# kawshik8/GAN-Image-Captioning

Measured on AMD Instinct MI355X. Metric: captions/sec (G+D train step), higher is better.
Workload: dtype bf16

## Files before the change

### gan-image-captioning_amd/csrc/gemm.hip

```cpp
#include "gemm.h"
#include "conv3x3.h"
#include "conv1x1_stream.h"
#include "conv1x1_panel.h"
#include "conv1x1_pix.h"
#include "conv_stem.h"
#include "bn_fold.h"
#include "kernels.h"

#include <stdlib.h>

namespace gic {

namespace {

typedef __attribute__((address_space(3))) bf16x4 lds_bf16x4;
typedef unsigned int u32x4 __attribute__((ext_vector_type(4)));
typedef const __attribute__((address_space(1))) u32x4* gptr_u4;

__device__ __attribute__((aligned(16))) unsigned int g_zero16[4] = {0u, 0u, 0u, 0u};
typedef __attribute__((address_space(3))) void* lds_void_ptr;
typedef const __attribute__((address_space(1))) void* gbl_void_ptr;

#ifdef GIC_STAMPS
}
__device__ unsigned long long g_stamp[32];
namespace {
#define STAMP(i) do { if (tid == 0 && blockIdx.y == 0 && (blockIdx.x == 0 || blockIdx.x == gridDim.x - 1)) { \
  const int o_ = blockIdx.x == 0 ? 0 : 16; g_stamp[o_ + 2 * (i)] = __builtin_amdgcn_s_memtime(); g_stamp[o_ + 2 * (i) + 1] = __builtin_amdgcn_s_memrealtime(); } } while (0)
#define DBG d.dbg
#else
#define STAMP(i) do {} while (0)
#define DBG 0
#endif

template <typename T> struct GlobalPtr { typedef const __attribute__((address_space(1))) T* type; };

template <typename TI, typename TO, bool AKC, bool BKC, int BM, int BN, bool VEC, int EPI, bool CONV, bool PIPE>
__global__ __launch_bounds__(256) void gemm_kernel(const GemmDesc d, const int k_tiles_per_split) {
  static_assert(!CONV || (AKC && BKC && VEC), "the implicit-GEMM convolution loader is k-contiguous and vectorised");
  static_assert(!PIPE || (AKC && BKC && VEC), "the LDS-DMA pipeline needs k-contiguous 16-byte chunks");
  constexpr int SZ = sizeof(TI);
  constexpr int BK = 128 / SZ;
  constexpr int VE = 16 / SZ;
  constexpr int SA = PIPE ? 128 : (AKC ? 144 : BM * SZ + 16);
  constexpr int SB = PIPE ? 128 : (BKC ? 144 : BN * SZ + 16);
  constexpr int NSTAGE = PIPE ? 3 : 2;
  constexpr int A_BYTES = AKC ? BM * SA : BK * SA;
  constexpr int B_BYTES = BKC ? BN * SB : BK * SB;
  constexpr int BUF_BYTES = A_BYTES + B_BYTES;
  constexpr int TM = BM / 32, TN = BN / 32;
  constexpr int CA = BM / 32, CB = BN / 32;
  constexpr bool IS_BF16 = (SZ == 2);
  typedef typename GlobalPtr<TI>::type gptr_t;

  constexpr int EPI_BYTES = BM * (BN * (int)sizeof(TO) + 16) + 4 * (BN / 2) * 2 * 4;
  constexpr int SMEM_BYTES = NSTAGE * BUF_BYTES > EPI_BYTES ? NSTAGE * BUF_BYTES : EPI_BYTES;
  __shared__ __attribute__((aligned(16))) unsigned char smem[SMEM_BYTES];

  const int tid = threadIdx.x, lane = tid & 63, w = tid >> 6;
  STAMP(0);
  const int wr = w >> 1, wc = w & 1;
  const int lr = lane & 15, lg = lane >> 4;

  const int tiles_m = (d.M + BM - 1) / BM;
  const int nwg = gridDim.x;
  int bid = blockIdx.x;
// ... 382 lines not shown
        if (m >= M) continue;
        float v = d.alpha * acc[i][j][r] + bias;
        if constexpr (EPI == EPI_BNSTATS) {
          C[(long)m * d.ldc + n] = from_f32<TO>(v);
          st_s += v; st_q += v * v;
        } else if constexpr (EPI == EPI_PLAIN) {
          const long o = (long)m * d.ldc + n;
          if constexpr (sizeof(TO) == 4) {
            if (split) { atomicAdd((float*)&C[o], v); continue; }
          }
          if (d.accumulate) v += to_f32<TO>(C[o]);
          C[o] = from_f32<TO>(v);
        } else {
          const float x = to_f32<TI>(((const TI*)d.X)[(long)m * d.ldx + n]);
          const float sg = 1.f / (1.f + expf(-v));
          const float y = sg * fmaxf(v, 0.f) + (1.f - sg) * x;
          if (d.Hpre) d.Hpre[(long)m * d.ldh + n] = v;
          float keep = keep4[r];
          if (d.mask) keep = (float)d.mask[(long)m * d.ldmask + n];
          if (d.mask_out) d.mask_out[(long)m * d.ldmask_out + n] = (uint8_t)keep;
          C[(long)m * d.ldc + n] = from_f32<TO>(y * keep * d.keep_scale);
        }
      }
      if constexpr (EPI == EPI_BNSTATS) {
        st_s += __shfl_xor(st_s, 16, 64); st_q += __shfl_xor(st_q, 16, 64);
        st_s += __shfl_xor(st_s, 32, 64); st_q += __shfl_xor(st_q, 32, 64);
        float* st = d.stats + (long)(blockIdx.x % d.stats_nrep) * 2 * N;
        if (lg == 0) { atomicAdd(&st[n], st_s); atomicAdd(&st[N + n], st_q); }
      }
    }
  }
}

template <typename TO, int BN, int EPI, bool CONV, int NS, bool ABN = false, bool ARES = false, int AMAXK = (ARES ? 2048 : 1024)>
__global__ __launch_bounds__(512) void tile8_kernel(const GemmDesc d, const unsigned a_bytes, const unsigned b_bytes) {
  static_assert(!ARES || ABN, "the residual-on-load form extends the A-side BatchNorm");
  constexpr int BM = 128, BK = 64, NT = 512;
  constexpr int TM = 2, TN = BN / 32;
  constexpr int CA = BM * 8 / NT, CB = BN * 8 / NT;
  constexpr int NL = CA + CB + (ARES ? CA : 0);
  constexpr int A_BYTES = BM * 128, B_BYTES = BN * 128, R_BYTES = ARES ? A_BYTES : 0, STAGE = A_BYTES + B_BYTES + R_BYTES;
  constexpr int OSZ = sizeof(TO), OVE = 16 / OSZ, SC = BN * OSZ + 16;
  constexpr int EPI_BYTES = EPI == EPI_HIGHWAY ? BM * (BN + 4) * 4 : (EPI == EPI_GUMBELMAX ? 8 * BN * 4 : BM * SC + 8 * (BN / 2) * 2 * 4);
  constexpr int RING_BYTES = NS * STAGE > EPI_BYTES ? NS * STAGE : EPI_BYTES;
  constexpr int ABN_MAXK = AMAXK;
  constexpr int SMEM_BYTES = RING_BYTES + (ABN ? ABN_MAXK * 8 : 0) + (ARES ? ABN_MAXK * 8 : 0);
  constexpr unsigned OOB = 0x80000000u;
  static_assert(CB >= 1 && SMEM_BYTES <= 160 * 1024, "tile8 LDS budget");
  __shared__ __attribute__((aligned(16))) unsigned char smem[SMEM_BYTES];

  const int tid = threadIdx.x, lane = tid & 63, w = tid >> 6;
  STAMP(0);
  const int wr = w >> 1, wc = w & 1;
  const int lr = lane & 15, lg = lane >> 4;

  const int tiles_m = (d.M + BM - 1) / BM, tiles_n = (d.N + BN - 1) / BN;
  const int bid = xcd_run(blockIdx.x, gridDim.x);
  const int bm0 = (d.n_fast ? bid / tiles_n : bid % tiles_m) * BM;
  const int bn0 = (d.n_fast ? bid % tiles_n : bid / tiles_m) * BN;
  const int M = d.M, N = d.N, K = d.K;

  const __amdgpu_buffer_rsrc_t rsA = __builtin_amdgcn_make_buffer_rsrc((void*)d.A, 0, (int)a_bytes, 0x00020000);
  const __amdgpu_buffer_rsrc_t rsB = __builtin_amdgcn_make_buffer_rsrc((void*)d.B, 0, (int)b_bytes, 0x00020000);
  const __amdgpu_buffer_rsrc_t rsR = __builtin_amdgcn_make_buffer_rsrc((void*)(ARES ? d.res : d.A), 0, (int)a_bytes, 0x00020000);

  const int kc = ((tid & 7) ^ ((tid >> 4) & 7)) * 8;
  int a_off[CA], a_hi0[CA], a_wi0[CA];
  bool a_ok[CA];
  int cv_r = 0, cv_s = 0, cv_c = 0;
#pragma unroll
  for (int i = 0; i < CA; ++i) {
    const int m = bm0 + (tid >> 3) + i * 64;
    a_ok[i] = m < M;
    if constexpr (CONV) {
      const int mm = a_ok[i] ? m : 0;
      const int wo = mm % d.cWo, t = mm / d.cWo;
      const int ho = t % d.cHo, n = t / d.cHo;
      a_hi0[i] = a_ok[i] ? ho * d.cStride - d.cPad : -(1 << 28);
      a_wi0[i] = wo * d.cStride - d.cPad;
      a_off[i] = ((n * d.cH + a_hi0[i]) * d.cW + a_wi0[i]) * d.cCin;
    } else {
      a_hi0[i] = a_wi0[i] = 0;
      a_off[i] = m * (int)d.lda;
    }
  }
  if constexpr (CONV) {
    cv_c = kc % d.cCin;
    const int t = kc / d.cCin;
    cv_s = t % d.cKW;
    cv_r = t / d.cKW;
  }
  int b_off[CB];
  bool b_ok[CB];
#pragma unroll
  for (int i = 0; i < CB; ++i) {
    const int n = bn0 + (tid >> 3) + i * 64;
    b_ok[i] = n < N;
    b_off[i] = n * (int)d.ldb;
  }
  const int wbase = (tid & ~63) * 16;

  auto issue = [&](int kt, int st) {
    unsigned char* sA = smem + st * STAGE;
    unsigned char* sB = sA + A_BYTES;
    const int k = kt * BK + kc;
    const bool kok = k < K;
#pragma unroll
    for (int i = 0; i < CA; ++i) {
      unsigned voff;
      if constexpr (CONV) {
        const bool ok = (unsigned)(a_hi0[i] + cv_r) < (unsigned)d.cH & (unsigned)(a_wi0[i] + cv_s) < (unsigned)d.cW & kok;
        voff = ok ? (unsigned)(a_off[i] + (cv_r * d.cW + cv_s) * d.cCin + cv_c) * 2u : OOB;
      } else {
        voff = (a_ok[i] & kok) ? (unsigned)(a_off[i] + k) * 2u : OOB;
      }
      __builtin_amdgcn_raw_ptr_buffer_load_lds(rsA, (lds_void_ptr)(sA + i * (NT * 16) + wbase), 16, (int)voff, 0, 0, CONV ? GIC_TRUNK_NT : 0);
      if constexpr (ARES)
        __builtin_amdgcn_raw_ptr_buffer_load_lds(rsR, (lds_void_ptr)(sB + B_BYTES + i * (NT * 16) + wbase), 16, (int)voff, 0, 0, CONV ? GIC_TRUNK_NT : 0);
    }
#pragma unroll
    for (int i = 0; i < CB; ++i) {
      const unsigned voff = (b_ok[i] & kok) ? (unsigned)(b_off[i] + k) * 2u : OOB;
      __builtin_amdgcn_raw_ptr_buffer_load_lds(rsB, (lds_void_ptr)(sB + i * (NT * 16) + wbase), 16, (int)voff, 0, 0, 0);
    }
    if constexpr (CONV) {
      cv_c += BK;
      while (cv_c >= d.cCin) {
        cv_c -= d.cCin;
        if (++cv_s == d.cKW) { cv_s = 0; ++cv_r; }
      }
    }
  };

  float* coef = (float*)(smem + RING_BYTES);
  if constexpr (ABN) {
    const int Cn = CONV ? d.cCin : K;
    for (int c = tid; c < ABN_MAXK; c += NT) {
      float sc = 0.f, sh = 0.f;
      if (c < Cn) {
        float s1, s2;
        fold_replicas(d.in_stats, d.in_nrep, Cn, c, s1, s2);
        const float mean = s1 * d.in_inv_count;
        const float var = fmaxf(s2 * d.in_inv_count - mean * mean, 0.f);
        sc = d.in_gamma[c] * rsqrtf(var + 1e-5f);
        sh = d.in_beta[c] - mean * sc;
      }
      coef[2 * c] = sc; coef[2 * c + 1] = sh;
      if constexpr (ARES) {
        float rs = 1.f, rt = 0.f;
        if (d.res_stats && c < Cn) {
          float s1, s2;
          fold_replicas(d.res_stats, d.res_nrep, Cn, c, s1, s2);
          const float mean = s1 * d.res_inv_count;
          const float var = fmaxf(s2 * d.res_inv_count - mean * mean, 0.f);
          rs = d.res_gamma[c] * rsqrtf(var + 1e-5f);
// ... 27 lines not shown
        for (int i = 0; i < CA; ++i) {
          const bool ok = CONV ? ((unsigned)(a_hi0[i] + tr) < (unsigned)d.cH & (unsigned)(a_wi0[i] + ts) < (unsigned)d.cW) : a_ok[i];
          if (!ok) continue;
          bf16x8* p = (bf16x8*)(smem + st * STAGE + i * (NT * 16) + tid * 16);
          bf16x8 v = *p;
          if constexpr (ARES) {
            const bf16x8 r = *(const bf16x8*)(smem + st * STAGE + A_BYTES + B_BYTES + i * (NT * 16) + tid * 16);
#pragma unroll
            for (int e = 0; e < 8; ++e) v[e] = (bf16_t)fmaxf((float)v[e] * scl[e] + sft[e] + ((float)r[e] * rsc[e] + rsf[e]), 0.f);
            if (wb) *(bf16x8*)((bf16_t*)d.out_wb + (long)a_off[i] + k) = v;
          } else {
#pragma unroll
            for (int e = 0; e < 8; ++e) v[e] = (bf16_t)fmaxf((float)v[e] * scl[e] + sft[e], 0.f);
          }
          *p = v;
        }
      }
    }
  };

  f32x4 acc[TM][TN];
#pragma unroll
  for (int i = 0; i < TM; ++i)
#pragma unroll
    for (int j = 0; j < TN; ++j) acc[i][j] = (f32x4){0.f, 0.f, 0.f, 0.f};

  auto compute = [&](int st) {
    const unsigned char* sA = smem + st * STAGE;
    const unsigned char* sB = sA + A_BYTES;
    bf16x8 fa[2][TM], fb[2][TN];
#pragma unroll
    for (int ks = 0; ks < 2; ++ks) {
#pragma unroll
      for (int t = 0; t < TM; ++t) {
        const int row = wr * 32 + t * 16 + lr;
        fa[ks][t] = *(const bf16x8*)(sA + row * 128 + (((ks * 4 + lg) ^ ((row >> 1) & 7)) << 4));
      }
#pragma unroll
      for (int t = 0; t < TN; ++t) {
        const int row = wc * (BN / 2) + t * 16 + lr;
        fb[ks][t] = *(const bf16x8*)(sB + row * 128 + (((ks * 4 + lg) ^ ((row >> 1) & 7)) << 4));
      }
    }
#pragma unroll
    for (int ks = 0; ks < 2; ++ks)
#pragma unroll
      for (int i = 0; i < TM; ++i)
#pragma unroll
        for (int j = 0; j < TN; ++j)
          acc[i][j] = __builtin_amdgcn_mfma_f32_16x16x32_bf16(fa[ks][i], fb[ks][j], acc[i][j], 0, 0, 0);
  };

  auto read_half = [&](int st, int ks, bf16x8 (&fa)[TM], bf16x8 (&fb)[TN]) {
    const unsigned char* sA = smem + st * STAGE;
    const unsigned char* sB = sA + A_BYTES;
#pragma unroll
    for (int t = 0; t < TM; ++t) {
      const int row = wr * 32 + t * 16 + lr;
      fa[t] = *(const bf16x8*)(sA + row * 128 + (((ks * 4 + lg) ^ ((row >> 1) & 7)) << 4));
    }
#pragma unroll
    for (int t = 0; t < TN; ++t) {
      const int row = wc * (BN / 2) + t * 16 + lr;
      fb[t] = *(const bf16x8*)(sB + row * 128 + (((ks * 4 + lg) ^ ((row >> 1) & 7)) << 4));
    }
  };
  auto mfma_half = [&](const bf16x8 (&fa)[TM], const bf16x8 (&fb)[TN]) {
#pragma unroll
    for (int i = 0; i < TM; ++i)
#pragma unroll
      for (int j = 0; j < TN; ++j)
        acc[i][j] = __builtin_amdgcn_mfma_f32_16x16x32_bf16(fa[i], fb[j], acc[i][j], 0, 0, 0);
  };

  const int nk = (K + BK - 1) / BK;
  STAMP(1);
  if constexpr (NS == 1) {
    for (int kt = 0; kt < nk; ++kt) {
      if (kt) __builtin_amdgcn_s_barrier();
      issue(kt, 0);
      asm volatile("s_waitcnt vmcnt(0)" ::: "memory");
      abn(kt, 0);
      __builtin_amdgcn_s_barrier();
      compute(0);
    }
  } else if constexpr (NS < 4) {
    issue(0, 0);
    int st = 0;
    for (int kt = 0; kt < nk; ++kt) {
      asm volatile("s_waitcnt vmcnt(0)" ::: "memory");
      abn(kt, st);
      __builtin_amdgcn_s_barrier();
      if (kt == 0) STAMP(2);
      if (!(DBG & 1)) issue(kt + 1, st ^ 1);
      if (!(DBG & 2)) compute(st);
      st ^= 1;
    }
  } else {
#pragma unroll
    for (int s = 0; s < NS - 1; ++s) issue(s, s);
    bf16x8 fa0[TM], fb0[TN], fa1[TM], fb1[TN];
    int st = 0, st_fill = NS - 1;
    for (int kt = 0; kt < nk; ++kt) {
      asm volatile("s_waitcnt vmcnt(%0) lgkmcnt(0)" ::"n"(NS >= 2 ? (NS - 2) * NL : 0) : "memory");
      abn(kt, st);
      __builtin_amdgcn_s_barrier();
      if (kt == 0) STAMP(2);
      if (!(DBG & 2)) {
        read_half(st, 0, fa0, fb0);
        __builtin_amdgcn_sched_barrier(0);
        if (kt > 0) mfma_half(fa1, fb1);
        __builtin_amdgcn_sched_barrier(0);
      }
      if (!(DBG & 1)) issue(kt + NS - 1, st_fill);
      if (!(DBG & 2)) {
        __builtin_amdgcn_sched_barrier(0);
        read_half(st, 1, fa1, fb1);
        __builtin_amdgcn_sched_barrier(0);
        mfma_half(fa0, fb0);
      }
      st = st == NS - 1 ? 0 : st + 1;
      st_fill = st_fill == NS - 1 ? 0 : st_fill + 1;
    }
    if (!(DBG & 2) && nk > 0) mfma_half(fa1, fb1);
  }
  asm volatile("s_waitcnt vmcnt(0)" ::: "memory");
  __syncthreads();
  STAMP(3);

  if constexpr (EPI == EPI_GUMBELMAX) {
    float* sV = (float*)smem;
    int* sI = (int*)(smem + 4 * BN * 4);
    const float eps = 1e-10f;
    const uint64_t seed = d.seed_dev ? *d.seed_dev : d.seed;
    const float T = d.gm_temperature;
#pragma unroll
    for (int j = 0; j < TN; ++j) {
      const int nl = wc * (BN / 2) + j * 16 + lr;
      const int n = bn0 + nl;
      float best = -INFINITY;
      int best_i = 0x7fffffff;
#pragma unroll
      for (int i = 0; i < TM; ++i) {
        const int m0 = bm0 + wr * 32 + i * 16 + lg * 4;
        if (m0 < M && n < N) {
          const float4 bv = *(const float4*)(d.gm_bias + m0);
          const float bia[4] = {bv.x, bv.y, bv.z, bv.w};
// ... 115 lines not shown
        if (!d.mask && d.use_philox) {
          uint32_t r0, r1, r2, r3;
          Philox::gen4(d.seed_dev ? *d.seed_dev : d.seed, d.stream, (uint64_t)(mb >> 2) * (uint64_t)N + (uint64_t)n, r0, r1, r2, r3);
          keep4[0] = Philox::u01(r0) >= d.drop_p ? 1.f : 0.f;
          keep4[1] = Philox::u01(r1) >= d.drop_p ? 1.f : 0.f;
          keep4[2] = Philox::u01(r2) >= d.drop_p ? 1.f : 0.f;
          keep4[3] = Philox::u01(r3) >= d.drop_p ? 1.f : 0.f;
        }
#pragma unroll
        for (int r = 0; r < 4; ++r) {
          const int m = mb + r;
          if (m >= M) continue;
          const float v = d.alpha * acc[i][j][r] + bias;
          const float x = to_f32<bf16_t>(((const bf16_t*)d.X)[(long)m * d.ldx + n]);
          const float sg = 1.f / (1.f + expf(-v));
          const float y = sg * fmaxf(v, 0.f) + (1.f - sg) * x;
          if (d.Hpre) d.Hpre[(long)m * d.ldh + n] = v;
          float keep = keep4[r];
          if (d.mask) keep = (float)d.mask[(long)m * d.ldmask + n];
          if (d.mask_out) d.mask_out[(long)m * d.ldmask_out + n] = (uint8_t)keep;
          C[(long)m * d.ldc + n] = from_f32<TO>(y * keep * d.keep_scale);
        }
      }
    }
    STAMP(5);
    return;
  }
  unsigned char* sC = smem;
  float* sStat = (float*)(smem + BM * SC);
#pragma unroll
  for (int j = 0; j < TN; ++j) {
    const int nl = wc * (BN / 2) + j * 16 + lr;
    const int n = bn0 + nl;
    const float bias = (d.bias && n < N) ? d.bias[n] : 0.f;
    float st_s = 0.f, st_q = 0.f;
#pragma unroll
    for (int i = 0; i < TM; ++i) {
#pragma unroll
      for (int r = 0; r < 4; ++r) {
        const int ml = wr * 32 + i * 16 + lg * 4 + r;
        const float v = d.alpha * acc[i][j][r] + bias;
        *(TO*)(sC + ml * SC + nl * OSZ) = from_f32<TO>(v);
        if (EPI == EPI_BNSTATS && bm0 + ml < M) { st_s += v; st_q += v * v; }
      }
    }
    if constexpr (EPI == EPI_BNSTATS) {
      st_s += __shfl_xor(st_s, 16, 64); st_q += __shfl_xor(st_q, 16, 64);
      st_s += __shfl_xor(st_s, 32, 64); st_q += __shfl_xor(st_q, 32, 64);
      if (lg == 0) { sStat[(w * (BN / 2) + j * 16 + lr) * 2] = st_s; sStat[(w * (BN / 2) + j * 16 + lr) * 2 + 1] = st_q; }
    }
  }
  __syncthreads();
  STAMP(4);
  if constexpr (EPI == EPI_BNSTATS) {
    if (tid < BN) {
      const int cwc = tid / (BN / 2), cl = tid % (BN / 2), n = bn0 + tid;
      if (n < N) {
        float s0 = 0.f, q0 = 0.f;
#pragma unroll
        for (int r = 0; r < 4; ++r) {
          s0 += sStat[((r * 2 + cwc) * (BN / 2) + cl) * 2];
          q0 += sStat[((r * 2 + cwc) * (BN / 2) + cl) * 2 + 1];
        }
        float* stp = d.stats + (long)(blockIdx.x % d.stats_nrep) * 2 * N;
        atomicAdd(&stp[n], s0);
        atomicAdd(&stp[N + n], q0);
      }
    }
  }
  constexpr int CPR = BN / OVE;
  for (int c = tid; c < BM * CPR; c += NT) {
    const int ml = c / CPR, cc = c % CPR;
    const int m = bm0 + ml, n = bn0 + cc * OVE;
    if (m < M && n < N) {
      u32x4 v = *(const u32x4*)(sC + ml * SC + cc * 16);
      if (d.accumulate) {
        const u32x4 o = *(const u32x4*)(C + (long)m * d.ldc + n);
        TO* pv = (TO*)&v;
        const TO* po = (const TO*)&o;
#pragma unroll
        for (int e = 0; e < OVE; ++e) pv[e] = from_f32<TO>(to_f32<TO>(pv[e]) + to_f32<TO>(po[e]));
      }
      *(u32x4*)(C + (long)m * d.ldc + n) = v;
    }
  }
  STAMP(5);
}

template <typename TO, int EPI, bool CONV>
bool try_tile8(const GemmDesc& d_in, hipStream_t stream) {
  static const bool off = getenv("GIC_NO_TILE8") != nullptr;
  GemmDesc d = d_in;
  constexpr int OVE = 16 / (int)sizeof(TO);
  if (off || d.M < 128) return false;
  if (EPI != EPI_HIGHWAY && ((d.N % OVE) || (d.ldc % OVE) || (((uintptr_t)d.C) & 15))) return false;
  if (EPI == EPI_HIGHWAY && d.in_dtype != DT_BF16) return false;
  if (!CONV && ((long)cdiv(d.M, 128) * cdiv(d.N, 64) < 128 || d.K < 256)) return false;
  const long a_elems = CONV ? (long)(d.M / (d.cHo * d.cWo)) * d.cH * d.cW * d.cCin : (long)(d.M - 1) * d.lda + d.K;
  const long b_elems = (long)(d.N - 1) * d.ldb + d.K;
  if (a_elems * 2 >= (1l << 31) || b_elems * 2 >= (1l << 31)) return false;
// ... 24 lines not shown
      } else {
        if (res_ns == 1) {
          if (n128) hipLaunchKernelGGL((tile8_kernel<TO, 128, EPI, CONV, 1, true, true, 2048>), grid, block, 0, stream, d, ab, bb);
          else hipLaunchKernelGGL((tile8_kernel<TO, 64, EPI, CONV, 1, true, true, 2048>), grid, block, 0, stream, d, ab, bb);
        } else {
          if (n128) hipLaunchKernelGGL((tile8_kernel<TO, 128, EPI, CONV, 2, true, true, 2048>), grid, block, 0, stream, d, ab, bb);
          else hipLaunchKernelGGL((tile8_kernel<TO, 64, EPI, CONV, 2, true, true, 2048>), grid, block, 0, stream, d, ab, bb);
        }
      }
      return true;
    }
    if (d.in_stats) {
      if (d.cCin % 8 || d.cCin > 1024 || !d.in_gamma || !d.in_beta || d.in_inv_count <= 0.f) return false;
      const int nk = cdiv(d.K, 64);
      const bool n128 = d.N >= 128 && big_tiles >= big_min;
      const long tiles = n128 ? big_tiles : (long)cdiv(d.M, 128) * cdiv(d.N, 64);
      const dim3 grid((unsigned)tiles), block(512);
      if (nk <= 4 && tiles > 512) {
        if (n128) hipLaunchKernelGGL((tile8_kernel<TO, 128, EPI, CONV, 1, true>), grid, block, 0, stream, d, ab, bb);
        else hipLaunchKernelGGL((tile8_kernel<TO, 64, EPI, CONV, 1, true>), grid, block, 0, stream, d, ab, bb);
      } else if (tiles > 256) {
        if (n128) hipLaunchKernelGGL((tile8_kernel<TO, 128, EPI, CONV, 2, true>), grid, block, 0, stream, d, ab, bb);
        else hipLaunchKernelGGL((tile8_kernel<TO, 64, EPI, CONV, 2, true>), grid, block, 0, stream, d, ab, bb);
      } else {
        if (n128) hipLaunchKernelGGL((tile8_kernel<TO, 128, EPI, CONV, 4, true>), grid, block, 0, stream, d, ab, bb);
        else hipLaunchKernelGGL((tile8_kernel<TO, 64, EPI, CONV, 4, true>), grid, block, 0, stream, d, ab, bb);
      }
      return true;
    }
  }
  static const int ns1_nk = [] { const char* e = getenv("GIC_TILE8_NS1_NK"); return e ? atoi(e) : 4; }();
  const int nk8 = cdiv(d.K, 64);
  if (EPI != EPI_HIGHWAY && nk8 <= ns1_nk && (d.N >= 128 ? big_tiles : (long)cdiv(d.M, 128) * cdiv(d.N, 64)) > 512) {
    if (d.N >= 128) hipLaunchKernelGGL((tile8_kernel<TO, 128, EPI, CONV, 1>), dim3((unsigned)big_tiles), dim3(512), 0, stream, d, ab, bb);
    else hipLaunchKernelGGL((tile8_kernel<TO, 64, EPI, CONV, 1>), dim3((unsigned)(cdiv(d.M, 128) * cdiv(d.N, 64))), dim3(512), 0, stream, d, ab, bb);
    return true;
  }
  if (d.N >= 128 && big_tiles >= big_min) {
    if (big_tiles > ns2_tiles) hipLaunchKernelGGL((tile8_kernel<TO, 128, EPI, CONV, 2>), dim3((unsigned)big_tiles), dim3(512), 0, stream, d, ab, bb);
    else hipLaunchKernelGGL((tile8_kernel<TO, 128, EPI, CONV, 4>), dim3((unsigned)big_tiles), dim3(512), 0, stream, d, ab, bb);
  } else {
    const long tiles = (long)cdiv(d.M, 128) * cdiv(d.N, 64);
    if (tiles > ns2_tiles) hipLaunchKernelGGL((tile8_kernel<TO, 64, EPI, CONV, 2>), dim3((unsigned)tiles), dim3(512), 0, stream, d, ab, bb);
    else hipLaunchKernelGGL((tile8_kernel<TO, 64, EPI, CONV, 4>), dim3((unsigned)tiles), dim3(512), 0, stream, d, ab, bb);
  }
  return true;
}


__global__ void zero2d_kernel(float* __restrict__ C, long ldc, int M, int N) {
  const long total = (long)M * N;
  for (long i = (long)blockIdx.x * blockDim.x + threadIdx.x; i < total; i += (long)gridDim.x * blockDim.x)
    C[(i / N) * ldc + (i % N)] = 0.f;
}

template <typename TI, typename TO, bool AKC, bool BKC, int BM, int BN, bool VEC, int EPI, bool CONV = false>
int launch(const GemmDesc& d, hipStream_t stream) {
  constexpr int BK = 128 / (int)sizeof(TI);
  const int tiles = cdiv(d.M, BM) * cdiv(d.N, BN);
  const int nk = cdiv(d.K, BK);
  int splits = 1;
  if (EPI == EPI_PLAIN && sizeof(TI) == 2 && sizeof(TO) == 4 && !d.no_split) {
    if (tiles < 24 && nk >= 8) {
      splits = 256 / tiles;
      if (splits > nk / 2) splits = nk / 2;
      if (splits > 16) splits = 16;
    } else if (tiles <= 192 && nk >= 32) {
      splits = 512 / tiles;
      if (splits > nk / 8) splits = nk / 8;
      if (splits > 16) splits = 16;
    } else if (!AKC && !BKC && tiles <= 192 && nk >= 16) {
      splits = 512 / tiles;
      if (splits > nk / 4) splits = nk / 4;
    } else if (tiles <= 320 && nk >= 64) {
      splits = 768 / tiles;
    }
    if (splits < 1) splits = 1;
    if (det_mode()) splits = (d.accumulate || splits < 2) ? 1 : 2;
  }
  int per = cdiv(nk, splits);
  splits = cdiv(nk, per);
  if (splits > 1 && !d.accumulate && !d.c_zeroed) {
    const long total = (long)d.M * d.N;
    const int g = (int)((total + 255) / 256 > 1024 ? 1024 : (total + 255) / 256);
    hipLaunchKernelGGL(zero2d_kernel, dim3(g), dim3(256), 0, stream, (float*)d.C, d.ldc, d.M, d.N);
  }
  constexpr bool CAN_PIPE = AKC && BKC && VEC;
  static const bool no_pipe = getenv("GIC_GEMM_NO_PIPE") != nullptr;
  const bool pipe = CAN_PIPE && per >= 6 && (long)tiles * splits <= 2 * 256 + 8 && !no_pipe;
  if constexpr (CAN_PIPE) {
    if (pipe) {
      hipLaunchKernelGGL((gemm_kernel<TI, TO, AKC, BKC, BM, BN, VEC, EPI, CONV, true>), dim3(tiles, splits), dim3(256), 0, stream, d, per);
      GIC_CHECK_LAUNCH("gemm");
      return GIC_OK;
    }
  }
  hipLaunchKernelGGL((gemm_kernel<TI, TO, AKC, BKC, BM, BN, VEC, EPI, CONV, false>), dim3(tiles, splits), dim3(256), 0, stream, d, per);
  GIC_CHECK_LAUNCH("gemm");
  return GIC_OK;
}

int big_tile_min() {
  static const int v = [] { const char* e = getenv("GIC_GEMM_BIG_MIN"); return e ? atoi(e) : 192; }();
  return v;
}

template <typename TI, typename TO, bool AKC, bool BKC, int EPI>
int pick_tile(const GemmDesc& d, bool vec, hipStream_t stream) {
  const long big_tiles = (long)cdiv(d.M, 128) * cdiv(d.N, 128);
  const bool big = big_tiles >= big_tile_min() && d.M >= 128 && d.N >= 128;
  if (big) {
    return vec ? launch<TI, TO, AKC, BKC, 128, 128, true, EPI>(d, stream)
               : launch<TI, TO, AKC, BKC, 128, 128, false, EPI>(d, stream);
  }
  return vec ? launch<TI, TO, AKC, BKC, 64, 64, true, EPI>(d, stream)
             : launch<TI, TO, AKC, BKC, 64, 64, false, EPI>(d, stream);
}

template <typename TI, typename TO, int EPI>
int pick_layout(const GemmDesc& d, bool vec, hipStream_t stream) {
  if constexpr (sizeof(TI) == 2) {
    if (d.a_kc && d.b_kc && vec && try_tile8<TO, EPI, false>(d, stream)) { GIC_CHECK_LAUNCH("gemm tile8"); return GIC_OK; }
  }
  if (d.a_kc && d.b_kc) return pick_tile<TI, TO, true, true, EPI>(d, vec, stream);
  if constexpr (EPI == EPI_PLAIN) {
    if (d.a_kc && !d.b_kc) return pick_tile<TI, TO, true, false, EPI>(d, vec, stream);
    if (!d.a_kc && !d.b_kc) return pick_tile<TI, TO, false, false, EPI>(d, vec, stream);
  }
  set_last_error("gemm: unsupported layout a_kc=%d b_kc=%d epi=%d", d.a_kc, d.b_kc, d.epi);
  return GIC_ERR_UNSUPPORTED;
}

template <typename TI, typename TO, int EPI>
int pick_conv(const GemmDesc& d, hipStream_t stream) {
  if constexpr (sizeof(TI) == 2 && sizeof(TO) == 2 && EPI == EPI_BNSTATS) {
    if (try_conv_stem(d, stream)) { GIC_CHECK_LAUNCH("conv stem"); return GIC_OK; }
    if (try_conv3x3_patch(d, stream)) { GIC_CHECK_LAUNCH("conv3x3 patch"); return GIC_OK; }
    if (try_conv1x1_stream(d, stream)) { GIC_CHECK_LAUNCH("conv1x1 stream"); return GIC_OK; }
    if (d.stats_only) return GIC_ERR_UNSUPPORTED;
    if (try_conv1x1_pix(d, stream)) { GIC_CHECK_LAUNCH("conv1x1 pix"); return GIC_OK; }
    if (try_conv1x1_panel(d, stream)) { GIC_CHECK_LAUNCH("conv1x1 panel"); return GIC_OK; }
    if (d.in_stats && d.cKH * d.cKW > 1) return GIC_ERR_UNSUPPORTED;
  }
  if constexpr (sizeof(TI) == 2) {
    if (try_tile8<TO, EPI, true>(d, stream)) { GIC_CHECK_LAUNCH("conv tile8"); return GIC_OK; }
  }
  if (d.in_stats) return GIC_ERR_UNSUPPORTED;
  const long big_tiles = (long)cdiv(d.M, 128) * cdiv(d.N, 128);
  if (big_tiles >= big_tile_min() && d.N >= 128) return launch<TI, TO, true, true, 128, 128, true, EPI, true>(d, stream);
  return launch<TI, TO, true, true, 64, 64, true, EPI, true>(d, stream);
}

template <typename TI, typename TO>
int pick_epi(const GemmDesc& d, bool vec, hipStream_t stream) {
  if (d.conv) {
    if (!vec || !d.a_kc || !d.b_kc) { set_last_error("gemm: convolution needs 16-B aligned NHWC / KRSC operands"); return GIC_ERR_UNSUPPORTED; }
    if constexpr (sizeof(TI) == sizeof(TO)) {
      if (d.epi == EPI_BNSTATS) return pick_conv<TI, TO, EPI_BNSTATS>(d, stream);
// ... 9 lines not shown
}

bool aligned16(const void* p) { return (((uintptr_t)p) & 15) == 0; }

}

int gemm_gumbelmax(const GemmDesc& d0, hipStream_t stream) {
  GemmDesc d = d0;
  static const bool off = getenv("GIC_NO_TILE8") != nullptr || getenv("GIC_NO_FUSED_GUMBELMAX") != nullptr;
  GIC_CHECK_ARG(d.A && d.B && d.gm_rowkey && d.gm_bias, "gemm_gumbelmax: null operand");
  if (off || d.in_dtype != DT_BF16 || !d.a_kc || !d.b_kc || d.M < 128 || d.M % 4 || d.K % 8 || d.lda % 8 || d.ldb % 8 || !aligned16(d.A) ||
      !aligned16(d.B) || !aligned16(d.gm_bias) || (d.gm_u && (!aligned16(d.gm_u) || d.gm_ldu % 4)) || !(d.gm_temperature > 0.f))
    return GIC_ERR_UNSUPPORTED;
  const long a_elems = (long)(d.M - 1) * d.lda + d.K, b_elems = (long)(d.N - 1) * d.ldb + d.K;
  const long tiles = (long)cdiv(d.M, 128) * cdiv(d.N, 128);
  if (a_elems * 2 >= (1l << 31) || b_elems * 2 >= (1l << 31) || d.N < 128 || tiles < 160) return GIC_ERR_UNSUPPORTED;
  d.epi = EPI_GUMBELMAX;
  d.n_fast = xcd_share_a(2l * d.M * d.K, 2l * d.N * d.K, cdiv(d.N, 128));
  const unsigned ab = (unsigned)(a_elems * 2), bb = (unsigned)(b_elems * 2);
  if (tiles > 256) hipLaunchKernelGGL((tile8_kernel<float, 128, EPI_GUMBELMAX, false, 2>), dim3((unsigned)tiles), dim3(512), 0, stream, d, ab, bb);
  else hipLaunchKernelGGL((tile8_kernel<float, 128, EPI_GUMBELMAX, false, 4>), dim3((unsigned)tiles), dim3(512), 0, stream, d, ab, bb);
  GIC_CHECK_LAUNCH("gemm gumbelmax");
  return GIC_OK;
}

int gemm(const GemmDesc& d0, hipStream_t stream) {
  GemmDesc d = d0;
#ifdef GIC_STAMPS
  { const char* e = getenv("GIC_GEMM_DBG"); if (e) d.dbg = atoi(e); }
#endif
  GIC_CHECK_ARG(d.A && d.B && d.C, "gemm: null operand");
  GIC_CHECK_ARG(d.M >= 0 && d.N >= 0 && d.K >= 0, "gemm: negative dim");
  if (d.M == 0 || d.N == 0) return GIC_OK;
  {
    static const bool log = getenv("GIC_GEMM_LOG") != nullptr;
    if (log && !d.conv)
      fprintf(stderr, "[gemm] M=%d N=%d K=%d a_kc=%d b_kc=%d in=%d out=%d epi=%d acc=%d\n", d.M, d.N, d.K, d.a_kc, d.b_kc, d.in_dtype, d.out_dtype, d.epi,
              d.accumulate);
  }
  if (d.epi == EPI_HIGHWAY) GIC_CHECK_ARG(d.X, "gemm: highway epilogue needs X");
  const int sz = dtype_size(d.in_dtype);
  const int ve = 16 / sz;
  bool vec = aligned16(d.A) && aligned16(d.B) && (d.lda % ve == 0) && (d.ldb % ve == 0);
  if (d.conv) {
    const bool chunk_ok = (d.cCin % ve == 0) || (d.cPad == 0 && ve % d.cCin == 0 && (d.cKW * d.cCin) % ve == 0);
    GIC_CHECK_ARG(chunk_ok && d.K == d.cKH * d.cKW * d.cCin && d.K % ve == 0, "gemm: conv needs Cin %% %d == 0 (or a pre-padded NHWC4 stem) and K = KH*KW*Cin", ve);
    GIC_CHECK_ARG(d.epi != EPI_BNSTATS || d.stats, "gemm: EPI_BNSTATS needs a stats buffer");
    vec = aligned16(d.A) && aligned16(d.B) && (d.ldb % ve == 0);
  }
  if (d.a_kc || d.b_kc) vec = vec && (d.K % ve == 0);
  if (d.in_dtype == DT_F32 && d.out_dtype == DT_F32) return pick_epi<float, float>(d, vec, stream);
  if (d.in_dtype == DT_BF16 && d.out_dtype == DT_F32) return pick_epi<bf16_t, float>(d, vec, stream);
  if (d.in_dtype == DT_BF16 && d.out_dtype == DT_BF16) return pick_epi<bf16_t, bf16_t>(d, vec, stream);
  set_last_error("gemm: unsupported dtypes in=%d out=%d", d.in_dtype, d.out_dtype);
  return GIC_ERR_UNSUPPORTED;
}

}
#ifdef GIC_STAMPS
extern "C" int gic_debug_stamps(unsigned long long* out) {
  return (int)hipMemcpyFromSymbol(out, HIP_SYMBOL(gic::g_stamp), sizeof(unsigned long long) * 32);
}
#endif
```

Measured before the change: 26590.

## Route transposed-operand bf16 GEMMs through tile8 kernel with LDS transpose reads and split-K

Extends the 512-thread tile8 MFMA kernel so it can take m- or n-contiguous (non-k-contiguous) A/B operands. It loads k-rows via buffer-to-LDS DMA with a swizzle and builds fragments with ds_read_tr16 transpose reads. Plain bf16 GEMMs with a transposed B (the backward-pass weight and input gradients) now use this kernel instead of the older 256-thread gemm_kernel. It also adds split-K over gridDim.y with fp32 atomic accumulation and a zero-fill pre-pass, which adds atomic traffic and may change results under non-deterministic ordering. Kernel-choice logging is added as well.

```diff
diff --git a/gan-image-captioning_amd/csrc/gemm.hip b/gan-image-captioning_amd/csrc/gemm.hip
--- a/gan-image-captioning_amd/csrc/gemm.hip
+++ b/gan-image-captioning_amd/csrc/gemm.hip
@@ -32,6 +32,9 @@
 #define STAMP(i) do {} while (0)
 #define DBG 0
 #endif
+
+struct GemmChoice { const char* kern; int bm, bn, splits, ns; };
+thread_local GemmChoice g_choice;
 
 template <typename T> struct GlobalPtr { typedef const __attribute__((address_space(1))) T* type; };
 
@@ -480,12 +483,37 @@
   }
 }
 
-template <typename TO, int BN, int EPI, bool CONV, int NS, bool ABN = false, bool ARES = false, int AMAXK = (ARES ? 2048 : 1024)>
+template <int CPR>
+__device__ __forceinline__ int tsw(const int kr) {
+  static_assert(CPR == 16 || CPR == 8, "128- or 64-row images");
+  return CPR == 16 ? (((kr & 3) << 2) | ((kr >> 2) & 3)) : ((kr & 2) | ((kr >> 1) & 4));
+}
+
+template <bool KC, int ROWS>
+__device__ __forceinline__ bf16x8 tile8_frag(const unsigned char* s, const int row0, const int ks, const int lr, const int lg) {
+  if constexpr (KC) {
+    const int row = row0 + lr;
+    return *(const bf16x8*)(s + row * 128 + (((ks * 4 + lg) ^ ((row >> 1) & 7)) << 4));
+  } else {
+    constexpr int RB = ROWS * 2;
+    const int q = lr >> 2, p = lr & 3;
+    const int c = (row0 >> 3) + (p >> 1);
+    const int k0 = ks * 32 + lg * 8 + q, k1 = k0 + 4;
+    const bf16x4 t0 = __builtin_amdgcn_ds_read_tr16_b64_v4bf16((lds_bf16x4*)(s + k0 * RB + ((c ^ tsw<ROWS / 8>(k0)) << 4) + 8 * (p & 1)));
+    const bf16x4 t1 = __builtin_amdgcn_ds_read_tr16_b64_v4bf16((lds_bf16x4*)(s + k1 * RB + ((c ^ tsw<ROWS / 8>(k1)) << 4) + 8 * (p & 1)));
+    return __builtin_shufflevector(t0, t1, 0, 1, 2, 3, 4, 5, 6, 7);
+  }
+}
+
+template <typename TO, int BN, int EPI, bool CONV, int NS, bool ABN = false, bool ARES = false, int AMAXK = (ARES ? 2048 : 1024),
+          bool AKC = true, bool BKC = true>
 __global__ __launch_bounds__(512) void tile8_kernel(const GemmDesc d, const unsigned a_bytes, const unsigned b_bytes) {
   static_assert(!ARES || ABN, "the residual-on-load form extends the A-side BatchNorm");
+  static_assert((AKC && BKC) || (EPI == EPI_PLAIN && !CONV && !ABN), "m/n-contiguous operands: plain products only");
   constexpr int BM = 128, BK = 64, NT = 512;
   constexpr int TM = 2, TN = BN / 32;
   constexpr int CA = BM * 8 / NT, CB = BN * 8 / NT;
+  constexpr int CPRA = BM / 8, CPRB = BN / 8;
   constexpr int NL = CA + CB + (ARES ? CA : 0);
   constexpr int A_BYTES = BM * 128, B_BYTES = BN * 128, R_BYTES = ARES ? A_BYTES : 0, STAGE = A_BYTES + B_BYTES + R_BYTES;
   constexpr int OSZ = sizeof(TO), OVE = 16 / OSZ, SC = BN * OSZ + 16;
@@ -507,6 +535,10 @@
   const int bm0 = (d.n_fast ? bid / tiles_n : bid % tiles_m) * BM;
   const int bn0 = (d.n_fast ? bid % tiles_n : bid / tiles_m) * BN;
   const int M = d.M, N = d.N, K = d.K;
+  const int nk_all = (K + BK - 1) / BK, per = (nk_all + (int)gridDim.y - 1) / (int)gridDim.y;
+  const int kt0 = (int)blockIdx.y * per;
+  const int nk = max(0, min(nk_all, kt0 + per) - kt0);
+  const int kend = min(K, (kt0 + nk) * BK);
 
   const __amdgpu_buffer_rsrc_t rsA = __builtin_amdgcn_make_buffer_rsrc((void*)d.A, 0, (int)a_bytes, 0x00020000);
   const __amdgpu_buffer_rsrc_t rsB = __builtin_amdgcn_make_buffer_rsrc((void*)d.B, 0, (int)b_bytes, 0x00020000);
@@ -518,6 +550,13 @@
   int cv_r = 0, cv_s = 0, cv_c = 0;
 #pragma unroll
   for (int i = 0; i < CA; ++i) {
+    if constexpr (!AKC) {
+      const int kr = (tid >> 4) + i * (NT / CPRA), m = bm0 + ((tid & 15) ^ tsw<CPRA>(kr)) * 8;
+      a_ok[i] = m < M;
+      a_hi0[i] = a_wi0[i] = 0;
+      a_off[i] = kr * (int)d.lda + m;
+      continue;
+    }
     const int m = bm0 + (tid >> 3) + i * 64;
     a_ok[i] = m < M;
     if constexpr (CONV) {
@@ -542,6 +581,12 @@
   bool b_ok[CB];
 #pragma unroll
   for (int i = 0; i < CB; ++i) {
+    if constexpr (!BKC) {
+      const int kr = tid / CPRB + i * (NT / CPRB), n = bn0 + ((tid % CPRB) ^ tsw<CPRB>(kr)) * 8;
+      b_ok[i] = n < N;
+      b_off[i] = kr * (int)d.ldb + n;
+      continue;
+    }
     const int n = bn0 + (tid >> 3) + i * 64;
     b_ok[i] = n < N;
     b_off[i] = n * (int)d.ldb;
@@ -552,11 +597,14 @@
     unsigned char* sA = smem + st * STAGE;
     unsigned char* sB = sA + A_BYTES;
     const int k = kt * BK + kc;
-    const bool kok = k < K;
+    const bool kok = k < kend;
 #pragma unroll
     for (int i = 0; i < CA; ++i) {
       unsigned voff;
-      if constexpr (CONV) {
+      if constexpr (!AKC) {
+        const bool ok = a_ok[i] & (kt * BK + (tid >> 4) + i * (NT / CPRA) < kend);
+        voff = ok ? ((unsigned)a_off[i] + (unsigned)(kt * BK) * (unsigned)d.lda) * 2u : OOB;
+      } else if constexpr (CONV) {
         const bool ok = (unsigned)(a_hi0[i] + cv_r) < (unsigned)d.cH & (unsigned)(a_wi0[i] + cv_s) < (unsigned)d.cW & kok;
         voff = ok ? (unsigned)(a_off[i] + (cv_r * d.cW + cv_s) * d.cCin + cv_c) * 2u : OOB;
       } else {
@@ -568,7 +616,13 @@
     }
 #pragma unroll
     for (int i = 0; i < CB; ++i) {
-      const unsigned voff = (b_ok[i] & kok) ? (unsigned)(b_off[i] + k) * 2u : OOB;
+      unsigned voff;
+      if constexpr (!BKC) {
+        const bool ok = b_ok[i] & (kt * BK + tid / CPRB + i * (NT / CPRB) < kend);
+        voff = ok ? ((unsigned)b_off[i] + (unsigned)(kt * BK) * (unsigned)d.ldb) * 2u : OOB;
+      } else {
+        voff = (b_ok[i] & kok) ? (unsigned)(b_off[i] + k) * 2u : OOB;
+      }
       __builtin_amdgcn_raw_ptr_buffer_load_lds(rsB, (lds_void_ptr)(sB + i * (NT * 16) + wbase), 16, (int)voff, 0, 0, 0);
     }
     if constexpr (CONV) {
@@ -662,15 +716,9 @@
 #pragma unroll
     for (int ks = 0; ks < 2; ++ks) {
 #pragma unroll
-      for (int t = 0; t < TM; ++t) {
-        const int row = wr * 32 + t * 16 + lr;
-        fa[ks][t] = *(const bf16x8*)(sA + row * 128 + (((ks * 4 + lg) ^ ((row >> 1) & 7)) << 4));
-      }
-#pragma unroll
-      for (int t = 0; t < TN; ++t) {
-        const int row = wc * (BN / 2) + t * 16 + lr;
-        fb[ks][t] = *(const bf16x8*)(sB + row * 128 + (((ks * 4 + lg) ^ ((row >> 1) & 7)) << 4));
-      }
+      for (int t = 0; t < TM; ++t) fa[ks][t] = tile8_frag<AKC, BM>(sA, wr * 32 + t * 16, ks, lr, lg);
+#pragma unroll
+      for (int t = 0; t < TN; ++t) fb[ks][t] = tile8_frag<BKC, BN>(sB, wc * (BN / 2) + t * 16, ks, lr, lg);
     }
 #pragma unroll
     for (int ks = 0; ks < 2; ++ks)
@@ -685,15 +733,9 @@
     const unsigned char* sA = smem + st * STAGE;
     const unsigned char* sB = sA + A_BYTES;
 #pragma unroll
-    for (int t = 0; t < TM; ++t) {
-      const int row = wr * 32 + t * 16 + lr;
-      fa[t] = *(const bf16x8*)(sA + row * 128 + (((ks * 4 + lg) ^ ((row >> 1) & 7)) << 4));
-    }
-#pragma unroll
-    for (int t = 0; t < TN; ++t) {
-      const int row = wc * (BN / 2) + t * 16 + lr;
-      fb[t] = *(const bf16x8*)(sB + row * 128 + (((ks * 4 + lg) ^ ((row >> 1) & 7)) << 4));
-    }
+    for (int t = 0; t < TM; ++t) fa[t] = tile8_frag<AKC, BM>(sA, wr * 32 + t * 16, ks, lr, lg);
+#pragma unroll
+    for (int t = 0; t < TN; ++t) fb[t] = tile8_frag<BKC, BN>(sB, wc * (BN / 2) + t * 16, ks, lr, lg);
   };
   auto mfma_half = [&](const bf16x8 (&fa)[TM], const bf16x8 (&fb)[TN]) {
 #pragma unroll
@@ -703,37 +745,36 @@
         acc[i][j] = __builtin_amdgcn_mfma_f32_16x16x32_bf16(fa[i], fb[j], acc[i][j], 0, 0, 0);
   };
 
-  const int nk = (K + BK - 1) / BK;
   STAMP(1);
   if constexpr (NS == 1) {
     for (int kt = 0; kt < nk; ++kt) {
       if (kt) __builtin_amdgcn_s_barrier();
-      issue(kt, 0);
+      issue(kt0 + kt, 0);
       asm volatile("s_waitcnt vmcnt(0)" ::: "memory");
-      abn(kt, 0);
+      abn(kt0 + kt, 0);
       __builtin_amdgcn_s_barrier();
       compute(0);
     }
   } else if constexpr (NS < 4) {
-    issue(0, 0);
+    issue(kt0, 0);
     int st = 0;
     for (int kt = 0; kt < nk; ++kt) {
       asm volatile("s_waitcnt vmcnt(0)" ::: "memory");
-      abn(kt, st);
+      abn(kt0 + kt, st);
       __builtin_amdgcn_s_barrier();
       if (kt == 0) STAMP(2);
-      if (!(DBG & 1)) issue(kt + 1, st ^ 1);
+      if (!(DBG & 1)) issue(kt0 + kt + 1, st ^ 1);
       if (!(DBG & 2)) compute(st);
       st ^= 1;
     }
   } else {
 #pragma unroll
-    for (int s = 0; s < NS - 1; ++s) issue(s, s);
+    for (int s = 0; s < NS - 1; ++s) issue(kt0 + s, s);
     bf16x8 fa0[TM], fb0[TN], fa1[TM], fb1[TN];
     int st = 0, st_fill = NS - 1;
     for (int kt = 0; kt < nk; ++kt) {
       asm volatile("s_waitcnt vmcnt(%0) lgkmcnt(0)" ::"n"(NS >= 2 ? (NS - 2) * NL : 0) : "memory");
-      abn(kt, st);
+      abn(kt0 + kt, st);
       __builtin_amdgcn_s_barrier();
       if (kt == 0) STAMP(2);
       if (!(DBG & 2)) {
@@ -742,7 +783,7 @@
         if (kt > 0) mfma_half(fa1, fb1);
         __builtin_amdgcn_sched_barrier(0);
       }
-      if (!(DBG & 1)) issue(kt + NS - 1, st_fill);
+      if (!(DBG & 1)) issue(kt0 + kt + NS - 1, st_fill);
       if (!(DBG & 2)) {
         __builtin_amdgcn_sched_barrier(0);
         read_half(st, 1, fa1, fb1);
@@ -924,7 +965,7 @@
   for (int j = 0; j < TN; ++j) {
     const int nl = wc * (BN / 2) + j * 16 + lr;
     const int n = bn0 + nl;
-    const float bias = (d.bias && n < N) ? d.bias[n] : 0.f;
+    const float bias = (d.bias && n < N && blockIdx.y == 0) ? d.bias[n] : 0.f;
     float st_s = 0.f, st_q = 0.f;
 #pragma unroll
     for (int i = 0; i < TM; ++i) {
@@ -958,6 +999,16 @@
         atomicAdd(&stp[n], s0);
         atomicAdd(&stp[N + n], q0);
       }
+    }
+  }
+  if constexpr (sizeof(TO) == 4) {
+    if (gridDim.y > 1) {
+      for (int e = tid; e < BM * BN; e += NT) {
+        const int ml = e / BN, nl = e % BN;
+        if (bm0 + ml < M && bn0 + nl < N) atomicAdd((float*)C + (long)(bm0 + ml) * d.ldc + bn0 + nl, *(const float*)(sC + ml * SC + nl * 4));
+      }
+      STAMP(5);
+      return;
     }
   }
   constexpr int CPR = BN / OVE;
@@ -1048,15 +1099,19 @@
   static const int ns1_nk = [] { const char* e = getenv("GIC_TILE8_NS1_NK"); return e ? atoi(e) : 4; }();
   const int nk8 = cdiv(d.K, 64);
   if (EPI != EPI_HIGHWAY && nk8 <= ns1_nk && (d.N >= 128 ? big_tiles : (long)cdiv(d.M, 128) * cdiv(d.N, 64)) > 512) {
+    g_choice = {"tile8", 128, d.N >= 128 ? 128 : 64, 1, 1};
     if (d.N >= 128) hipLaunchKernelGGL((tile8_kernel<TO, 128, EPI, CONV, 1>), dim3((unsigned)big_tiles), dim3(512), 0, stream, d, ab, bb);
     else hipLaunchKernelGGL((tile8_kernel<TO, 64, EPI, CONV, 1>), dim3((unsigned)(cdiv(d.M, 128) * cdiv(d.N, 64))), dim3(512), 0, stream, d, ab, bb);
     return true;
   }
+  g_choice = {"tile8", 128, d.N >= 128 && big_tiles >= big_min ? 128 : 64, 1, 0};
   if (d.N >= 128 && big_tiles >= big_min) {
+    g_choice.ns = big_tiles > ns2_tiles ? 2 : 4;
     if (big_tiles > ns2_tiles) hipLaunchKernelGGL((tile8_kernel<TO, 128, EPI, CONV, 2>), dim3((unsigned)big_tiles), dim3(512), 0, stream, d, ab, bb);
     else hipLaunchKernelGGL((tile8_kernel<TO, 128, EPI, CONV, 4>), dim3((unsigned)big_tiles), dim3(512), 0, stream, d, ab, bb);
   } else {
     const long tiles = (long)cdiv(d.M, 128) * cdiv(d.N, 64);
+    g_choice.ns = tiles > ns2_tiles ? 2 : 4;
     if (tiles > ns2_tiles) hipLaunchKernelGGL((tile8_kernel<TO, 64, EPI, CONV, 2>), dim3((unsigned)tiles), dim3(512), 0, stream, d, ab, bb);
     else hipLaunchKernelGGL((tile8_kernel<TO, 64, EPI, CONV, 4>), dim3((unsigned)tiles), dim3(512), 0, stream, d, ab, bb);
   }
@@ -1068,6 +1123,71 @@
   const long total = (long)M * N;
   for (long i = (long)blockIdx.x * blockDim.x + threadIdx.x; i < total; i += (long)gridDim.x * blockDim.x)
     C[(i / N) * ldc + (i % N)] = 0.f;
+}
+
+template <typename TO, bool AKC, bool BKC, int BN, int NS>
+void launch_tile8_t(const GemmDesc& d, const dim3 grid, const unsigned ab, const unsigned bb, hipStream_t stream) {
+  hipLaunchKernelGGL((tile8_kernel<TO, BN, EPI_PLAIN, false, NS, false, false, 1024, AKC, BKC>), grid, dim3(512), 0, stream, d, ab, bb);
+}
+
+template <typename TO, bool AKC>
+bool try_tile8_t(const GemmDesc& d_in, hipStream_t stream) {
+  static const bool off = getenv("GIC_NO_TILE8") != nullptr || getenv("GIC_NO_TILE8_T") != nullptr;
+  static const int ns1_nk = [] { const char* e = getenv("GIC_TILE8_NS1_NK"); return e ? atoi(e) : 4; }();
+  static const int shallow_min = [] { const char* e = getenv("GIC_TILE8_T_SHALLOW_MIN"); return e ? atoi(e) : 256; }();
+  static const int deep_min = [] { const char* e = getenv("GIC_TILE8_T_MIN_BLOCKS"); return e ? atoi(e) : 128; }();
+  static const int min_per = [] { const char* e = getenv("GIC_TILE8_T_MIN_PER"); return e ? atoi(e) : 12; }();
+  static const int split_blocks = [] { const char* e = getenv("GIC_TILE8_T_SPLIT_BLOCKS"); return e ? atoi(e) : 256; }();
+  constexpr int OVE = 16 / (int)sizeof(TO);
+  GemmDesc d = d_in;
+  if (off || d.M < 128 || (d.N % OVE) || (d.ldc % OVE) || (((uintptr_t)d.C) & 15)) return false;
+  const long a_elems = AKC ? (long)(d.M - 1) * d.lda + d.K : (long)(d.K - 1) * d.lda + d.M;
+  const long b_elems = (long)(d.K - 1) * d.ldb + d.N;
+  if (a_elems * 2 >= (1l << 31) || b_elems * 2 >= (1l << 31)) return false;
+  const unsigned ab = (unsigned)(a_elems * 2), bb = (unsigned)(b_elems * 2);
+  const int nk = cdiv(d.K, 64), tiles_m = cdiv(d.M, 128);
+  int bn = 128, splits = 1, ns;
+  long tiles;
+  if (nk <= ns1_nk) {
+    bn = 64;
+    tiles = (long)tiles_m * cdiv(d.N, 64);
+    if (tiles < shallow_min) return false;
+    ns = 1;
+  } else {
+    auto plan = [&](int n_tile) {
+      tiles = (long)tiles_m * cdiv(d.N, n_tile);
+      splits = 1;
+      if (sizeof(TO) == 4 && !d.no_split && tiles < split_blocks) {
+        splits = (int)(split_blocks / tiles);
+        if (splits > nk / min_per) splits = nk / min_per;
+        if (splits > 16) splits = 16;
+        if (splits < 1) splits = 1;
+        if (det_mode()) splits = (d.accumulate || splits < 2) ? 1 : 2;
+        splits = cdiv(nk, cdiv(nk, splits));
+      }
+      return tiles * splits;
+    };
+    if (d.N < 128 || plan(128) < 192) bn = 64;
+    if (bn == 64 && plan(64) < deep_min) return false;
+    ns = tiles * splits > 256 ? 2 : 4;
+  }
+  if (splits > 1 && !d.accumulate && !d.c_zeroed) {
+    const long total = (long)d.M * d.N;
+    const int g = (int)((total + 255) / 256 > 1024 ? 1024 : (total + 255) / 256);
+    hipLaunchKernelGGL(zero2d_kernel, dim3(g), dim3(256), 0, stream, (float*)d.C, d.ldc, d.M, d.N);
+  }
+  d.n_fast = xcd_share_a(2l * d.M * d.K, 2l * d.N * d.K, cdiv(d.N, bn));
+  const dim3 grid((unsigned)tiles, (unsigned)splits);
+  g_choice = {"tile8", 128, bn, splits, ns};
+  if (bn == 128) {
+    if (ns == 4) launch_tile8_t<TO, AKC, false, 128, 4>(d, grid, ab, bb, stream);
+    else launch_tile8_t<TO, AKC, false, 128, 2>(d, grid, ab, bb, stream);
+  } else {
+    if (ns == 4) launch_tile8_t<TO, AKC, false, 64, 4>(d, grid, ab, bb, stream);
+    else if (ns == 2) launch_tile8_t<TO, AKC, false, 64, 2>(d, grid, ab, bb, stream);
+    else launch_tile8_t<TO, AKC, false, 64, 1>(d, grid, ab, bb, stream);
+  }
+  return true;
 }
 
 template <typename TI, typename TO, bool AKC, bool BKC, int BM, int BN, bool VEC, int EPI, bool CONV = false>
@@ -1104,6 +1224,7 @@
   constexpr bool CAN_PIPE = AKC && BKC && VEC;
   static const bool no_pipe = getenv("GIC_GEMM_NO_PIPE") != nullptr;
   const bool pipe = CAN_PIPE && per >= 6 && (long)tiles * splits <= 2 * 256 + 8 && !no_pipe;
+  g_choice = {pipe ? "gemm_kernel.pipe" : "gemm_kernel", BM, BN, splits, pipe ? 3 : 2};
   if constexpr (CAN_PIPE) {
     if (pipe) {
       hipLaunchKernelGGL((gemm_kernel<TI, TO, AKC, BKC, BM, BN, VEC, EPI, CONV, true>), dim3(tiles, splits), dim3(256), 0, stream, d, per);
@@ -1140,6 +1261,11 @@
   }
   if (d.a_kc && d.b_kc) return pick_tile<TI, TO, true, true, EPI>(d, vec, stream);
   if constexpr (EPI == EPI_PLAIN) {
+    if constexpr (sizeof(TI) == 2) {
+      if (!d.b_kc && vec) {
+        if (d.a_kc ? try_tile8_t<TO, true>(d, stream) : try_tile8_t<TO, false>(d, stream)) { GIC_CHECK_LAUNCH("gemm tile8 t"); return GIC_OK; }
+      }
+    }
     if (d.a_kc && !d.b_kc) return pick_tile<TI, TO, true, false, EPI>(d, vec, stream);
     if (!d.a_kc && !d.b_kc) return pick_tile<TI, TO, false, false, EPI>(d, vec, stream);
   }
@@ -1215,12 +1341,6 @@
   GIC_CHECK_ARG(d.A && d.B && d.C, "gemm: null operand");
   GIC_CHECK_ARG(d.M >= 0 && d.N >= 0 && d.K >= 0, "gemm: negative dim");
   if (d.M == 0 || d.N == 0) return GIC_OK;
-  {
-    static const bool log = getenv("GIC_GEMM_LOG") != nullptr;
-    if (log && !d.conv)
-      fprintf(stderr, "[gemm] M=%d N=%d K=%d a_kc=%d b_kc=%d in=%d out=%d epi=%d acc=%d\n", d.M, d.N, d.K, d.a_kc, d.b_kc, d.in_dtype, d.out_dtype, d.epi,
-              d.accumulate);
-  }
   if (d.epi == EPI_HIGHWAY) GIC_CHECK_ARG(d.X, "gemm: highway epilogue needs X");
   const int sz = dtype_size(d.in_dtype);
   const int ve = 16 / sz;
@@ -1232,11 +1352,22 @@
     vec = aligned16(d.A) && aligned16(d.B) && (d.ldb % ve == 0);
   }
   if (d.a_kc || d.b_kc) vec = vec && (d.K % ve == 0);
-  if (d.in_dtype == DT_F32 && d.out_dtype == DT_F32) return pick_epi<float, float>(d, vec, stream);
-  if (d.in_dtype == DT_BF16 && d.out_dtype == DT_F32) return pick_epi<bf16_t, float>(d, vec, stream);
-  if (d.in_dtype == DT_BF16 && d.out_dtype == DT_BF16) return pick_epi<bf16_t, bf16_t>(d, vec, stream);
-  set_last_error("gemm: unsupported dtypes in=%d out=%d", d.in_dtype, d.out_dtype);
-  return GIC_ERR_UNSUPPORTED;
+  g_choice = {"?", 0, 0, 1, 0};
+  int rc;
+  if (d.in_dtype == DT_F32 && d.out_dtype == DT_F32) rc = pick_epi<float, float>(d, vec, stream);
+  else if (d.in_dtype == DT_BF16 && d.out_dtype == DT_F32) rc = pick_epi<bf16_t, float>(d, vec, stream);
+  else if (d.in_dtype == DT_BF16 && d.out_dtype == DT_BF16) rc = pick_epi<bf16_t, bf16_t>(d, vec, stream);
+  else {
+    set_last_error("gemm: unsupported dtypes in=%d out=%d", d.in_dtype, d.out_dtype);
+    return GIC_ERR_UNSUPPORTED;
+  }
+  {
+    static const bool log = getenv("GIC_GEMM_LOG") != nullptr;
+    if (log && !d.conv)
+      fprintf(stderr, "[gemm] M=%d N=%d K=%d a_kc=%d b_kc=%d in=%d out=%d epi=%d acc=%d kernel=%s tile=%dx%d splits=%d ns=%d\n", d.M, d.N, d.K, d.a_kc,
+              d.b_kc, d.in_dtype, d.out_dtype, d.epi, d.accumulate, g_choice.kern, g_choice.bm, g_choice.bn, g_choice.splits, g_choice.ns);
+  }
+  return rc;
 }
 
 }
```

Result: no change. 26690, median of 6 (+0.4%).
